# taylorlu/voicepuppet

Measured on AMD Instinct MI355X. Metric: PixReferNet G+D step frames/sec @256x256 bs=32, higher is better.
Workload: dtype bf16; 1 GPU; PixReferNet G+D training step (G + 3xD + VGG16-conv3_3 perceptual + TF-Adam x2), 256x256, ngf=ndf=64, global batch 32 = 32 per GPU; global_batch=32, per_gpu_batch=32, parallelism=dp1

## Files before the change

### include/vp_hip.h

```cpp
#ifndef VP_HIP_H_
#define VP_HIP_H_

#include <stddef.h>
#include <stdint.h>

#ifdef __cplusplus
extern "C" {
#endif

enum vp_status { VP_OK = 0, VP_ERR_ARG = -1, VP_ERR_HIP = -2, VP_ERR_WORKSPACE = -3, VP_ERR_STATE = -4 };
enum vp_dtype { VP_F32 = 0, VP_BF16 = 1 };
enum vp_act { VP_ACT_NONE = 0, VP_ACT_LRELU = 1, VP_ACT_RELU = 2, VP_ACT_TANH = 3, VP_ACT_SIGMOID = 4, VP_ACT_RELU6 = 5, VP_ACT_LEAKY = 6 };

int vp_version(void);
const char* vp_last_error(void);

typedef struct vp_pixrefer_desc {
  int batch;
  int height;
  int ngf, ndf;
  int dtype;
  int training;
  float l1_weight;
  float gan_weight;
// ... 511 lines not shown
typedef struct vp_avimux vp_avimux_t;
size_t vp_avimux_workspace_bytes(const vp_avimux_desc* d);
size_t vp_avimux_out_capacity(const vp_avimux_desc* d);
size_t vp_avimux_table_bytes(const vp_avimux_desc* d, int frames);
int vp_avimux_create(const vp_avimux_desc* d, void* workspace, size_t workspace_bytes, vp_avimux_t** out);
int vp_avimux_segment(vp_avimux_t* h, const unsigned char* data, size_t row_bytes, const int* lengths, const int* frame_slot, int frames,
                      const float* pcm, const int* sample_offset, const int* sample_count, int samples, unsigned char* out, size_t out_capacity,
                      void* stream);
void vp_avimux_destroy(vp_avimux_t* h);

#define VP_TRIPTYCH_MAX_FRAMES 4096
#define VP_TRIPTYCH_MAX_SIZE 1024
typedef struct vp_triptych_desc {
  uint32_t struct_bytes;
  int32_t max_frames;
  int32_t size;
  int32_t face_size;
  int32_t max_side;
} vp_triptych_desc;
size_t vp_triptych_desc_size(void);
typedef struct vp_triptych vp_triptych_t;
size_t vp_triptych_workspace_bytes(const vp_triptych_desc* d);
int vp_triptych_create(const vp_triptych_desc* d, void* workspace, size_t workspace_bytes, void* stream, vp_triptych_t** out);
int vp_triptych_build(vp_triptych_t* h, const unsigned char* frames, const unsigned char* render, const unsigned char* face_mask, const int* geometry,
                      const unsigned char* alpha, int n, unsigned char* triptych, int* status, void* stream);
int vp_triptych_mask(vp_triptych_t* h, const unsigned char* face_mask, const int* geometry, int n, int fill, void* stream);
int vp_triptych_fill_holes(const unsigned char* masks, int n, int height, int width, unsigned char* out, void* stream);
int vp_triptych_blur_taps(int q[21]);
int vp_triptych_tensor(vp_triptych_t* h, const char* name, void** ptr, int64_t shape[4]);
void vp_triptych_destroy(vp_triptych_t* h);

#define VP_KEYMATTE_MAX_FRAMES 4096
#define VP_KEYMATTE_MAX_SIZE 1024
#define VP_KEYMATTE_MAX_RADIUS 16
#define VP_KEYMATTE_MODEL_DOUBLES 19
typedef struct vp_keymatte_desc {
  uint32_t struct_bytes;
  int32_t max_frames;
  int32_t max_height;
  int32_t max_width;
  int32_t max_radius;
} vp_keymatte_desc;
size_t vp_keymatte_desc_size(void);
typedef struct vp_keymatte vp_keymatte_t;
size_t vp_keymatte_workspace_bytes(const vp_keymatte_desc* d);
int vp_keymatte_create(const vp_keymatte_desc* d, void* workspace, size_t workspace_bytes, vp_keymatte_t** out);
void vp_keymatte_destroy(vp_keymatte_t* h);
int vp_keymatte_fit(vp_keymatte_t* h, const unsigned char* frames, size_t row_pitch, size_t frame_stride, int n, int height, int width,
                    int band, int side_rows, double trim, double sigma_min, void* stream);
int vp_keymatte_apply(vp_keymatte_t* h, const unsigned char* frames, size_t row_pitch, size_t frame_stride, int n, int height, int width,
                      double lo, double hi, int radius, double eps, unsigned char* raw, unsigned char* matte, void* stream);
int vp_keymatte_get_model(vp_keymatte_t* h, double* model, void* stream);
int vp_keymatte_set_model(vp_keymatte_t* h, const double* model, void* stream);
int vp_keymatte_tensor(vp_keymatte_t* h, const char* name, void** ptr, int64_t shape[4]);
int vp_keymatte_solve_host(const int64_t moments[21], double sigma_min, double* model);

int vp_key_foreground(vp_keymatte_t* h, const unsigned char* frames, size_t row_pitch, size_t frame_stride, int n, int height, int width,
                      const unsigned char* matte, double despill, unsigned char* out, void* stream);

#define VP_MATTECLEAN_MAX_FRAMES 4096
#define VP_MATTECLEAN_MAX_SIZE 1024
#define VP_MATTECLEAN_MAX_GROW 16
#define VP_MATTECLEAN_MAX_ANCHORS 256
#define VP_MATTECLEAN_REPORT_INTS 8
#define VP_MATTECLEAN_KEEP_ALL 0
#define VP_MATTECLEAN_KEEP_ANCHORED 1
typedef struct vp_matteclean_desc {
  uint32_t struct_bytes;
  int32_t max_frames;
  int32_t max_height;
  int32_t max_width;
} vp_matteclean_desc;
size_t vp_matteclean_desc_size(void);
typedef struct vp_matteclean vp_matteclean_t;
size_t vp_matteclean_workspace_bytes(const vp_matteclean_desc* d);
int vp_matteclean_create(const vp_matteclean_desc* d, void* workspace, size_t workspace_bytes, vp_matteclean_t** out);
void vp_matteclean_destroy(vp_matteclean_t* h);
int vp_matteclean_clean(vp_matteclean_t* h, const unsigned char* matte, int n, int height, int width, int support, int core, int min_area,
                        int max_hole, int grow, int keep, const int* anchors, int k, unsigned char* out, void* stream);
int vp_matteclean_tensor(vp_matteclean_t* h, const char* name, void** ptr, int64_t shape[4]);

unsigned vp_crc32c(const void* data, size_t n, unsigned crc);

#ifdef __cplusplus
}
#endif
#endif
```

### voicepuppet_amd/_lib.py

```python
import ctypes
import os

_HERE = os.path.dirname(os.path.abspath(__file__))
LIB_PATH = os.environ.get("VP_LIB", os.path.join(_HERE, "libvp_hip.so"))

VP_F32, VP_BF16 = 0, 1
ACT_NONE, ACT_LRELU, ACT_RELU, ACT_TANH, ACT_SIGMOID = 0, 1, 2, 3, 4
BN_PATH_PLANNER, BN_PATH_TWO_PASS, BN_PATH_ONE_LAUNCH = 0, 1, 2


class PixReferDesc(ctypes.Structure):
  _fields_ = [("batch", ctypes.c_int), ("height", ctypes.c_int), ("ngf", ctypes.c_int), ("ndf", ctypes.c_int),
              ("dtype", ctypes.c_int), ("training", ctypes.c_int), ("l1_weight", ctypes.c_float),
              ("gan_weight", ctypes.c_float), ("per_sample_bn", ctypes.c_int),
              ("streams", ctypes.c_int), ("d_backward_fork", ctypes.c_int), ("d_beside_vgg", ctypes.c_int)]


class ConvDesc(ctypes.Structure):
  _fields_ = [("kind", ctypes.c_int), ("n", ctypes.c_int), ("h", ctypes.c_int), ("w", ctypes.c_int),
              ("cin", ctypes.c_int), ("cout", ctypes.c_int), ("ksize", ctypes.c_int), ("stride", ctypes.c_int),
              ("pad", ctypes.c_int), ("dtype", ctypes.c_int), ("in_act", ctypes.c_int), ("out_act", ctypes.c_int)]


class LogMelDesc(ctypes.Structure):
# ... 67 lines not shown
  _fields_ = [("struct_bytes", ctypes.c_uint32), ("max_frames", ctypes.c_int32), ("max_height", ctypes.c_int32), ("max_width", ctypes.c_int32)]


FRAME_METRICS_MAX_FRAMES = 4096


class AviMuxDesc(ctypes.Structure):
  _fields_ = [("struct_bytes", ctypes.c_uint32), ("max_frames", ctypes.c_int32), ("row_bytes", ctypes.c_int32), ("slots", ctypes.c_int32),
              ("max_samples", ctypes.c_int32)]


AVIMUX_MAX_FRAMES, AVIMUX_MAX_SLOTS = 4096, 128


class KeyMatteDesc(ctypes.Structure):
  _fields_ = [("struct_bytes", ctypes.c_uint32), ("max_frames", ctypes.c_int32), ("max_height", ctypes.c_int32), ("max_width", ctypes.c_int32),
              ("max_radius", ctypes.c_int32)]


KEYMATTE_MAX_FRAMES, KEYMATTE_MAX_SIZE, KEYMATTE_MAX_RADIUS, KEYMATTE_MODEL_DOUBLES = 4096, 1024, 16, 19


class MatteCleanDesc(ctypes.Structure):
  _fields_ = [("struct_bytes", ctypes.c_uint32), ("max_frames", ctypes.c_int32), ("max_height", ctypes.c_int32), ("max_width", ctypes.c_int32)]


MATTECLEAN_MAX_FRAMES, MATTECLEAN_MAX_SIZE, MATTECLEAN_MAX_GROW, MATTECLEAN_MAX_ANCHORS, MATTECLEAN_REPORT_INTS = 4096, 1024, 16, 256, 8
MATTECLEAN_KEEP_ALL, MATTECLEAN_KEEP_ANCHORED = 0, 1


class TriptychDesc(ctypes.Structure):
  _fields_ = [("struct_bytes", ctypes.c_uint32), ("max_frames", ctypes.c_int32), ("size", ctypes.c_int32), ("face_size", ctypes.c_int32),
              ("max_side", ctypes.c_int32)]


TRIPTYCH_MAX_FRAMES, TRIPTYCH_MAX_SIZE = 4096, 1024


class BfmObserveOpts(ctypes.Structure):
  _fields_ = [("struct_bytes", ctypes.c_uint32), ("visibility", ctypes.c_int32), ("raster_scale", ctypes.c_int32), ("prefilter", ctypes.c_int32),
              ("depth_tol", ctypes.c_float)]


class BfmModel(ctypes.Structure):
  _fields_ = [("nver", ctypes.c_int), ("ntri", ctypes.c_int), ("meanshape", ctypes.c_void_p), ("idBase", ctypes.c_void_p),
              ("exBase", ctypes.c_void_p), ("meantex", ctypes.c_void_p), ("texBase", ctypes.c_void_p), ("tri", ctypes.c_void_p),
              ("point_buf", ctypes.c_void_p), ("center", ctypes.c_double * 3), ("focal", ctypes.c_double),
              ("image_center", ctypes.c_double), ("sh", ctypes.c_double * 5)]


_P = ctypes.c_void_p
_SIGNATURES = {
    "vp_version": (ctypes.c_int, []),
    "vp_last_error": (ctypes.c_char_p, []),
    "vp_pixrefer_param_count": (ctypes.c_size_t, [ctypes.POINTER(PixReferDesc), ctypes.c_int]),
    "vp_pixrefer_param_info": (ctypes.c_int, [ctypes.POINTER(PixReferDesc), ctypes.c_int, ctypes.c_int, ctypes.c_char_p,
                                              ctypes.c_int, ctypes.POINTER(ctypes.c_size_t), ctypes.POINTER(ctypes.c_int),
                                              ctypes.POINTER(ctypes.c_int64)]),
    "vp_pixrefer_workspace_bytes": (ctypes.c_size_t, [ctypes.POINTER(PixReferDesc)]),
    "vp_pixrefer_validate_plan": (ctypes.c_int, [ctypes.POINTER(PixReferDesc)]),
    "vp_pixrefer_create": (ctypes.c_int, [ctypes.POINTER(PixReferDesc), _P, ctypes.c_size_t, _P, _P, _P, _P, _P, _P,
                                          ctypes.POINTER(_P)]),
    "vp_pixrefer_destroy": (None, [_P]),
    "vp_pixrefer_params_changed": (ctypes.c_int, [_P]),
    "vp_pixrefer_optimizer_stepped": (ctypes.c_int, [_P]),
    "vp_pixrefer_forward": (ctypes.c_int, [_P, _P, _P, _P, _P, _P]),
    "vp_pixrefer_forward_fg3": (ctypes.c_int, [_P, _P, _P, _P, _P]),
    "vp_pixrefer_desc_size": (ctypes.c_size_t, []),
    "vp_pixrefer_backward": (ctypes.c_int, [_P, _P]),
    "vp_pixrefer_backward_update": (ctypes.c_int, [_P, _P, _P, _P, _P, ctypes.c_int, ctypes.c_int, ctypes.c_float, ctypes.c_float,
                                                   ctypes.c_float, ctypes.c_float, _P]),
    "vp_pixrefer_backward_d": (ctypes.c_int, [_P, _P]),
    "vp_pixrefer_backward_g": (ctypes.c_int, [_P, _P]),
    "vp_pixrefer_backward_d_fork": (ctypes.c_int, [_P, _P]),
    "vp_pixrefer_backward_d_join": (ctypes.c_int, [_P, _P]),
    "vp_pixrefer_backward_g_stages": (ctypes.c_int, []),
    "vp_pixrefer_backward_g_stage": (ctypes.c_int, [_P, ctypes.c_int, _P]),
    "vp_pixrefer_side_stream": (ctypes.c_void_p, [_P]),
    "vp_pixrefer_use_streams": (ctypes.c_int, [_P, ctypes.c_int]),
    "vp_pixrefer_set_option": (ctypes.c_int, [_P, ctypes.c_char_p, ctypes.c_int]),
    "vp_pixrefer_fetch": (ctypes.c_int, [_P, ctypes.c_int, _P, _P]),
    "vp_pixrefer_counter": (ctypes.c_longlong, [_P, ctypes.c_char_p]),
    "vp_crc32c": (ctypes.c_uint, [_P, ctypes.c_size_t, ctypes.c_uint]),
    "vp_pixrefer_phase_ms": (ctypes.c_int, [_P, ctypes.POINTER(ctypes.c_float), ctypes.c_int]),
    "vp_grad_pack_bf16": (ctypes.c_int, [_P, _P, ctypes.c_size_t, _P]),
    "vp_grad_unpack_bf16": (ctypes.c_int, [_P, _P, ctypes.c_size_t, ctypes.c_float, _P]),
    "vp_pixrefer_update_bucket": (ctypes.c_int, [_P, ctypes.c_int, ctypes.c_int, _P, _P, ctypes.c_int, ctypes.c_float, ctypes.c_float, ctypes.c_float,
                                                 ctypes.c_float, _P]),
    "vp_resize_paste_workspace_bytes": (ctypes.c_size_t, [ctypes.c_int, ctypes.c_int]),
    "vp_resize_paste_u8": (ctypes.c_int, [_P, ctypes.c_int, ctypes.c_int, ctypes.c_int, ctypes.c_int, ctypes.c_int, ctypes.c_int, _P, ctypes.c_int,
                                          ctypes.c_int, ctypes.c_int, ctypes.c_int, _P, _P]),
    "vp_resize_linear_table": (ctypes.c_int, [ctypes.c_int, ctypes.c_int, ctypes.c_int, _P, _P, _P, _P]),
    "vp_mm_workspace_bytes": (ctypes.c_size_t, [ctypes.c_int, ctypes.c_int, ctypes.c_int]),
    "vp_mm_fwd_f32": (ctypes.c_int, [_P, ctypes.c_int, _P, ctypes.c_int, ctypes.c_int, _P, _P, ctypes.c_int, ctypes.c_int, ctypes.c_int, ctypes.c_int, _P, _P]),
    "vp_mm_bwd_data_f32": (ctypes.c_int, [_P, ctypes.c_int, _P, ctypes.c_int, ctypes.c_int, _P, ctypes.c_int, ctypes.c_int, ctypes.c_int, ctypes.c_int,
                                          ctypes.c_int, _P, _P]),
    "vp_mm_bwd_weight_f32": (ctypes.c_int, [_P, ctypes.c_int, _P, ctypes.c_int, _P, ctypes.c_int, ctypes.c_int, ctypes.c_int, ctypes.c_int, _P, _P]),
    "vp_mm_packed_bytes": (ctypes.c_size_t, [ctypes.c_int, ctypes.c_int, ctypes.c_int, ctypes.c_int]),
    "vp_mm_pack_desc_bytes": (ctypes.c_size_t, []),
    "vp_mm_pack_desc": (ctypes.c_int, [ctypes.c_size_t, ctypes.c_int, ctypes.c_int, ctypes.c_int, ctypes.c_int, ctypes.c_int, ctypes.c_int, ctypes.c_size_t, _P]),
    "vp_mm_pack_table": (ctypes.c_int, [_P, ctypes.c_int, _P, _P, _P]),
    "vp_mm_fwd_f32_packed": (ctypes.c_int, [_P, ctypes.c_int, _P, _P, _P, ctypes.c_int, ctypes.c_int, ctypes.c_int, ctypes.c_int, _P, _P]),
    "vp_mm_bwd_data_f32_packed": (ctypes.c_int, [_P, ctypes.c_int, _P, _P, ctypes.c_int, ctypes.c_int, ctypes.c_int, ctypes.c_int, ctypes.c_int, _P, _P]),
    "vp_pixrefer_mark_ms": (ctypes.c_float, [_P, ctypes.c_int, ctypes.c_int]),
    "vp_profile_enable": (ctypes.c_int, [ctypes.c_int]),
    "vp_tune": (ctypes.c_int, [ctypes.c_char_p, ctypes.c_int]),
    "vp_reserve_streams": (ctypes.c_int, []),
    "vp_host_stream": (ctypes.c_void_p, []),
    "vp_pixrefer_pack_frames": (ctypes.c_int, [_P, _P, _P, ctypes.c_int, ctypes.c_int, _P, _P, _P, _P, _P]),
    "vp_profile_collect": (ctypes.c_size_t, [ctypes.c_char_p, ctypes.c_size_t]),
    "vp_pixrefer_tensor": (ctypes.c_int, [_P, ctypes.c_char_p, ctypes.POINTER(_P), ctypes.POINTER(ctypes.c_int64),
                                          ctypes.POINTER(ctypes.c_int)]),
    "vp_adam_tf": (ctypes.c_int, [_P, _P, _P, _P, ctypes.c_size_t, ctypes.c_int, ctypes.c_float, ctypes.c_float,
                                  ctypes.c_float, ctypes.c_float, _P]),
    "vp_conv_workspace_bytes": (ctypes.c_size_t, [ctypes.POINTER(ConvDesc)]),
    "vp_conv_fwd": (ctypes.c_int, [ctypes.POINTER(ConvDesc), _P, _P, _P, _P, _P, _P, _P, _P]),
    "vp_conv_bwd_data": (ctypes.c_int, [ctypes.POINTER(ConvDesc), _P, _P, _P, _P, _P]),
    "vp_conv_bwd_weight": (ctypes.c_int, [ctypes.POINTER(ConvDesc), _P, _P, _P, _P, _P, _P, _P]),
    "vp_conv3x3_c64_bwd_data_pooled_workspace_bytes": (ctypes.c_size_t, [ctypes.POINTER(ConvDesc)]),
    "vp_conv3x3_c64_bwd_data_pooled": (ctypes.c_int, [ctypes.POINTER(ConvDesc), _P, _P, _P, _P, _P, _P, ctypes.c_int, _P]),
    "vp_bn_workspace_bytes": (ctypes.c_size_t, [ctypes.c_int, ctypes.c_int, ctypes.c_int]),
    "vp_bn_stats": (ctypes.c_int, [_P, ctypes.c_int, ctypes.c_int, ctypes.c_int, _P, _P, ctypes.c_float, _P, _P, _P, _P, _P, _P]),
    "vp_logmel_workspace_bytes": (ctypes.c_size_t, [ctypes.POINTER(LogMelDesc)]),
    "vp_logmel_frames": (ctypes.c_int, [ctypes.POINTER(LogMelDesc)]),
    "vp_logmel_create": (ctypes.c_int, [ctypes.POINTER(LogMelDesc), _P, ctypes.c_size_t, _P, ctypes.POINTER(_P)]),
    "vp_logmel_destroy": (None, [_P]),
    "vp_logmel_forward": (ctypes.c_int, [_P, _P, _P, _P]),
    "vp_bfmnet_param_count": (ctypes.c_size_t, []),
    "vp_bfmnet_param_info": (ctypes.c_int, [ctypes.c_int, ctypes.c_char_p, ctypes.c_int, ctypes.POINTER(ctypes.c_size_t),
                                            ctypes.POINTER(ctypes.c_int), ctypes.POINTER(ctypes.c_int64)]),
    "vp_bfmnet_workspace_bytes": (ctypes.c_size_t, [ctypes.POINTER(BfmNetDesc)]),
    "vp_bfmnet_create": (ctypes.c_int, [ctypes.POINTER(BfmNetDesc), _P, ctypes.c_size_t, _P, _P, ctypes.POINTER(_P)]),
    "vp_bfmnet_destroy": (None, [_P]),
    "vp_bfmnet_params_changed": (ctypes.c_int, [_P]),
    "vp_bfmnet_forward": (ctypes.c_int, [_P, _P, _P, _P, _P, _P]),
    "vp_bfmnet_set_decoder_dropout": (ctypes.c_int, [_P, _P, _P]),
    "vp_bfmnet_tensor": (ctypes.c_int, [_P, ctypes.c_char_p, ctypes.POINTER(_P), ctypes.POINTER(ctypes.c_int64)]),
    "vp_bfmstream_desc_size": (ctypes.c_size_t, []),
    "vp_bfmstream_context": (ctypes.c_int, [ctypes.POINTER(BfmStreamDesc)] + [ctypes.POINTER(ctypes.c_int)] * 5),
    "vp_bfmstream_frames_after": (ctypes.c_longlong, [ctypes.POINTER(BfmStreamDesc), ctypes.c_longlong, ctypes.c_int]),
    "vp_bfmstream_workspace_bytes": (ctypes.c_size_t, [ctypes.POINTER(BfmStreamDesc)]),
    "vp_bfmstream_create": (ctypes.c_int, [ctypes.POINTER(BfmStreamDesc), _P, ctypes.c_size_t, _P, _P, ctypes.POINTER(_P)]),
    "vp_bfmstream_destroy": (None, [_P]),
    "vp_bfmstream_params_changed": (ctypes.c_int, [_P]),
    "vp_bfmstream_reset": (ctypes.c_int, [_P, _P]),
    "vp_bfmstream_ready": (ctypes.c_int, [_P, ctypes.c_longlong]),
    "vp_bfmstream_ready_finish": (ctypes.c_int, [_P]),
    "vp_bfmstream_push": (ctypes.c_int, [_P, _P, ctypes.c_longlong, _P, _P, _P]),
    "vp_bfmstream_finish": (ctypes.c_int, [_P, _P, _P, _P]),
    "vp_bfmstream_tensor": (ctypes.c_int, [_P, ctypes.c_char_p, ctypes.POINTER(_P), ctypes.POINTER(ctypes.c_int64)]),
    "vp_bfmstream_group_desc_size": (ctypes.c_size_t, []),
    "vp_puppet_desc_size": (ctypes.c_size_t, []),
    "vp_puppet_workspace_bytes": (ctypes.c_size_t, [ctypes.POINTER(PuppetDesc)]),
    "vp_puppet_create": (ctypes.c_int, [ctypes.POINTER(PuppetDesc), _P, ctypes.c_size_t, _P, ctypes.POINTER(_P)]),
    "vp_puppet_destroy": (None, [_P]),
    "vp_puppet_attach": (ctypes.c_int, [_P, ctypes.c_int, _P, _P, _P, ctypes.c_int, ctypes.c_int, ctypes.c_int, _P]),
    "vp_puppet_set_backgrounds": (ctypes.c_int, [_P, _P, ctypes.c_int]),
    "vp_puppet_splice": (ctypes.c_int, [_P, _P, ctypes.c_int, _P, ctypes.c_int, _P, _P]),
    "vp_puppet_condition": (ctypes.c_int, [_P, _P, ctypes.c_int, _P, ctypes.c_int, _P, _P, _P, _P]),
    "vp_puppet_tensor": (ctypes.c_int, [_P, ctypes.c_char_p, ctypes.POINTER(_P), ctypes.POINTER(ctypes.c_int64)]),
    "vp_puppet_slot_info": (ctypes.c_int, [_P, ctypes.c_int, ctypes.POINTER(ctypes.c_int)]),
    "vp_jpeg_desc_size": (ctypes.c_size_t, []),
    "vp_jpeg_workspace_bytes": (ctypes.c_size_t, [ctypes.POINTER(JpegDesc)]),
    "vp_jpeg_frame_capacity": (ctypes.c_size_t, [ctypes.POINTER(JpegDesc)]),
    "vp_jpeg_create": (ctypes.c_int, [ctypes.POINTER(JpegDesc), _P, ctypes.c_size_t, _P, ctypes.POINTER(_P)]),
    "vp_jpeg_encode": (ctypes.c_int, [_P, _P, ctypes.c_int, _P, ctypes.c_size_t, _P, _P]),
# ... 236 lines not shown
```

### voicepuppet_amd/csrc/wgrad_tr.hip

```cpp
#include <stdlib.h>

#include "conv_ops.h"
#include "igemm_device.h"
#include "launch.h"

namespace vp {

__device__ __forceinline__ int tr_swz(int p) { return ((p & 3) | (((p >> 3) & 1) << 2)) << 1; }

typedef short v4s16 __attribute__((ext_vector_type(4)));

template <int ROWB>
__device__ __forceinline__ uint4 tr_frag8(const char* __restrict__ stage, int off) {
  typedef __attribute__((address_space(3))) v4s16 lds_v4;
  const v4s16 lo = __builtin_amdgcn_ds_read_tr16_b64_v4i16((lds_v4*)(stage + off));
  const v4s16 hi = __builtin_amdgcn_ds_read_tr16_b64_v4i16((lds_v4*)(stage + off + 4 * ROWB));
  union { v4s16 v[2]; uint4 u; } f;
  f.v[0] = lo; f.v[1] = hi;
  return f.u;
}

struct TrTask {
  const bf16* base;
  int C;
  int s, dh, dw;
  int Hs, Ws;
  int p;
  bool ok;
};

__device__ __forceinline__ TrTask tr_task(const PixSrc& src, int ch, bool ok, int s, int dh, int dw, int Hs, int Ws, int p, const void* zeros) {
  TrTask t;
  const bool second = ch >= src.C[0];
  t.C = second ? src.C[1] : src.C[0];
  t.base = reinterpret_cast<const bf16*>(second ? src.ptr[1] : src.ptr[0]) + (second ? ch - src.C[0] : ch);
  t.s = s; t.dh = dh; t.dw = dw; t.Hs = Hs; t.Ws = Ws; t.p = p; t.ok = ok;
  if (!ok) { t.base = reinterpret_cast<const bf16*>(zeros); t.C = 0; }
  return t;
}

__device__ __forceinline__ const void* tr_src(const WgradArgs& a, const TrTask& t, int it) {
  const int slot = it * 32 + t.p;
  const int r = slot & ((1 << a.lw) - 1), q = (slot >> a.lw) & ((1 << a.lh) - 1), n = slot >> (a.lw + a.lh);
  const int ih = q * t.s + t.dh, iw = r * t.s + t.dw;
  const bool ok = t.ok && n < a.N && q < a.Hb && r < a.Wb && (unsigned)ih < (unsigned)t.Hs && (unsigned)iw < (unsigned)t.Ws;
  return ok ? (const void*)(t.base + ((size_t)(n * t.Hs + ih) * t.Ws + iw) * t.C) : a.zeros;
}

template <int WM, int WN, int TC, int TP, int NST, bool FAST, bool EXACT = false>
__global__ __launch_bounds__(WM * WN * 64, (TC * TP > 16 ? 2 : 4)) void wgrad_tr_kernel(const WgradArgs a) {
  constexpr int NW = WM * WN;
  static_assert(NW == 8, "eight waves");
  constexpr int BM = WM * TC * 16, BN = WN * TP * 16;
  constexpr int PA = BM / 8, PB = BN / 8;
  constexpr int ASTG = 32 * PA, BSTG = 32 * PB, STG = ASTG + BSTG;
  constexpr int JA = ASTG / 64 / NW, JB = BSTG / 64 / NW;
  static_assert(JA * NW * 64 == ASTG && JB * NW * 64 == BSTG, "whole DMA instructions per wave");
  constexpr int J = JA + JB;
  extern __shared__ __attribute__((aligned(16))) char smem[];
  uint4* lds = reinterpret_cast<uint4*>(smem);

  const int tid = threadIdx.x, lane = tid & 63;
  const int wave = __builtin_amdgcn_readfirstlane(tid >> 6);
  int bx = blockIdx.x, by = blockIdx.y, bz = blockIdx.z;
  if (a.xcd_remap && (gridDim.z & 7) == 0) {
    const int ntile = gridDim.x * gridDim.y;
    const int L = bx + by * gridDim.x + bz * ntile;
    const int xcd = L & 7, j = L >> 3;
    bz = xcd + 8 * (j / ntile);
    const int t = j % ntile;
    bx = t % gridDim.x; by = t / gridDim.x;
  }
  const int m_base = bx * BM, d_base = by * BN, split = bz;
  const int niter = (a.N << (a.lw + a.lh)) / 32;
  const int per = (niter + a.splitk - 1) / a.splitk;
  const int it0 = split * per, it1 = min(niter, it0 + per);

  TrTask ta[JA], tb[JB];
#pragma unroll
  for (int j = 0; j < JA; ++j) {
    const int idx = (wave + NW * j) * 64 + lane;
    const int p = idx / PA, c = (idx % PA) ^ tr_swz(p);
    const int m = m_base + c * 8;
    const int tap = m >> a.log2Gc, ch = m & a.gc_mask;
    int tdh = 0, tdw = 0;
#pragma unroll
    for (int t = 0; t < 16; ++t) if (t == tap) { tdh = a.taps.dh[t]; tdw = a.taps.dw[t]; }
    ta[j] = tr_task(a.g, ch, tap < a.ntaps && ch < a.g.C[0] + a.g.C[1], a.s, tdh, tdw, a.Hgin, a.Wgin, p, a.zeros);
  }
#pragma unroll
  for (int j = 0; j < JB; ++j) {
    const int idx = (wave + NW * j) * 64 + lane;
    const int p = idx / PB, c = (idx % PB) ^ tr_swz(p);
    const int ch = d_base + c * 8;
    tb[j] = tr_task(a.d, ch, ch < a.Dc, 1, 0, 0, a.Hb, a.Wb, p, a.zeros);
  }
  const int W2 = 1 << a.lw;
  const bool gsecond = a.g.C[1] > 0 && (m_base & (a.Gc - 1)) >= a.g.C[0];
  const bool dsecond = a.d.C[1] > 0 && d_base >= a.d.C[0];
  const int gC = gsecond ? a.g.C[1] : a.g.C[0], dC = dsecond ? a.d.C[1] : a.d.C[0];
  constexpr bool fast = FAST;
  const unsigned gguard = (unsigned)((2 * a.Wgin + 2) * gC * 2);
  __amdgpu_buffer_rsrc_t rsG = make_rsrc((const char*)(gsecond ? a.g.ptr[1] : a.g.ptr[0]) - gguard,
                                         (unsigned)((size_t)a.N * a.Hgin * a.Wgin * gC * 2) + gguard);
  __amdgpu_buffer_rsrc_t rsD = make_rsrc(dsecond ? a.d.ptr[1] : a.d.ptr[0], (unsigned)((size_t)a.N * a.Hb * a.Wb * dC * 2));
  int fq[JA], fB[JA], fr[JA], fD[JA];
  unsigned fvo[JA];
  bool fok[JA];
  int bq[JB], br[JB];
  unsigned bvo[JB];
  bool bok[JB];
#pragma unroll
  for (int j = 0; j < JA; ++j) {
    const TrTask& t = ta[j];
    const int pq = W2 <= 32 ? t.p >> a.lw : 0, pr = W2 <= 32 ? t.p & (W2 - 1) : t.p;
    fq[j] = pq; fB[j] = pq * t.s + t.dh; fr[j] = pr; fD[j] = pr * t.s + t.dw;
    const int chl = (int)(t.base - reinterpret_cast<const bf16*>(gsecond ? a.g.ptr[1] : a.g.ptr[0]));
    fvo[j] = gguard + (unsigned)(((fB[j] * a.Wgin + fD[j]) * gC + chl) * 2);
    fok[j] = t.ok;
    if (EXACT && !t.ok) fvo[j] = DMA_OOB;
  }
#pragma unroll
  for (int j = 0; j < JB; ++j) {
    const TrTask& t = tb[j];
    bq[j] = W2 <= 32 ? t.p >> a.lw : 0; br[j] = W2 <= 32 ? t.p & (W2 - 1) : t.p;
    const int chl = (int)(t.base - reinterpret_cast<const bf16*>(dsecond ? a.d.ptr[1] : a.d.ptr[0]));
    bvo[j] = (unsigned)(((bq[j] * a.Wb + br[j]) * dC + chl) * 2);
    bok[j] = t.ok;
    if (EXACT && !t.ok) bvo[j] = DMA_OOB;
  }
  auto issue_fast = [&](int it, int stage) {
    uint4* la = lds + stage * STG;
    uint4* lb = la + ASTG;
    const int u = it * 32;
    const int ru = u & (W2 - 1), qu = (u >> a.lw) & ((1 << a.lh) - 1), nu = u >> (a.lw + a.lh);
    const bool nok = nu < a.N;
    const unsigned gso = (unsigned)((((nu * a.Hgin + qu * a.s) * a.Wgin + ru * a.s) * gC) * 2);
    const unsigned dso = (unsigned)((((nu * a.Hb + qu) * a.Wb + ru) * dC) * 2);
    const int qs = qu * a.s, rs = ru * a.s;
    if constexpr (EXACT) {
#pragma unroll
      for (int j = 0; j < JA; ++j) {
        const bool ok = (unsigned)(qs + fB[j]) < (unsigned)a.Hgin && (unsigned)(rs + fD[j]) < (unsigned)a.Wgin;
        dma16_buf(rsG, ok ? fvo[j] : DMA_OOB, gso, la + (wave + NW * j) * 64);
      }
#pragma unroll
      for (int j = 0; j < JB; ++j) dma16_buf(rsD, bvo[j], dso, lb + (wave + NW * j) * 64);
    } else {
#pragma unroll
      for (int j = 0; j < JA; ++j) {
        const bool ok = fok[j] && nok && qu + fq[j] < a.Hb && ru + fr[j] < a.Wb &&
                        (unsigned)(qs + fB[j]) < (unsigned)a.Hgin && (unsigned)(rs + fD[j]) < (unsigned)a.Wgin;
        dma16_buf(rsG, ok ? fvo[j] : DMA_OOB, gso, la + (wave + NW * j) * 64);
      }
#pragma unroll
      for (int j = 0; j < JB; ++j) {
        const bool ok = bok[j] && nok && qu + bq[j] < a.Hb && ru + br[j] < a.Wb;
        dma16_buf(rsD, ok ? bvo[j] : DMA_OOB, dso, lb + (wave + NW * j) * 64);
      }
    }
  };
  auto issue = [&](int it, int stage) {
    if constexpr (fast) { issue_fast(it, stage); return; }
    uint4* la = lds + stage * STG;
    uint4* lb = la + ASTG;
#pragma unroll
    for (int j = 0; j < JA; ++j) dma16(tr_src(a, ta[j], it), la + (wave + NW * j) * 64);
#pragma unroll
    for (int j = 0; j < JB; ++j) dma16(tr_src(a, tb[j], it), lb + (wave + NW * j) * 64);
  };

  const int wm = wave / WN, wn = wave - wm * WN;
  const int g = lane >> 4, t16 = lane & 15;
  const int fp = 8 * g + (t16 >> 2), q2 = t16 & 3, fsw = tr_swz(fp);
  int offA[TC], offB[TP];
#pragma unroll
  for (int tc = 0; tc < TC; ++tc) offA[tc] = fp * (BM * 2) + (((2 * (wm * TC + tc) + (q2 >> 1)) ^ fsw) << 4) + (q2 & 1) * 8;
#pragma unroll
  for (int tp = 0; tp < TP; ++tp) offB[tp] = ASTG * 16 + fp * (BN * 2) + (((2 * (wn * TP + tp) + (q2 >> 1)) ^ fsw) << 4) + (q2 & 1) * 8;

  f32x4 acc[TC][TP];
#pragma unroll
  for (int i = 0; i < TC; ++i)
#pragma unroll
    for (int j = 0; j < TP; ++j) acc[i][j] = (f32x4){0.f, 0.f, 0.f, 0.f};

  if (it0 < it1) {
#pragma unroll
    for (int dd = 0; dd < NST - 1; ++dd) if (it0 + dd < it1) issue(it0 + dd, dd);
    int st = 0;
    for (int it = it0; it < it1; ++it) {
      if (it + NST - 2 < it1) asm volatile("s_waitcnt vmcnt(%0)" ::"n"((NST - 2) * J) : "memory");
      else asm volatile("s_waitcnt vmcnt(0)" ::: "memory");
      __builtin_amdgcn_s_barrier();
      asm volatile("" ::: "memory");
      const int stn = st == 0 ? NST - 1 : st - 1;
      if (it + NST - 1 < it1) issue(it + NST - 1, stn);
      const char* stage = smem + (size_t)st * STG * 16;
      uint4 fa[TC], fb[TP];
#pragma unroll
      for (int tp = 0; tp < TP; ++tp) fb[tp] = tr_frag8<BN * 2>(stage, offB[tp]);
#pragma unroll
      for (int tc = 0; tc < TC; ++tc) fa[tc] = tr_frag8<BM * 2>(stage, offA[tc]);
#pragma unroll
      for (int tc = 0; tc < TC; ++tc)
#pragma unroll
        for (int tp = 0; tp < TP; ++tp) acc[tc][tp] = mma16<bf16>(fa[tc], fb[tp], acc[tc][tp]);
      st = st == NST - 1 ? 0 : st + 1;
    }
  }

  if (a.splitk == 1) {
#pragma unroll
    for (int tc = 0; tc < TC; ++tc)
#pragma unroll
      for (int tp = 0; tp < TP; ++tp) {
        const int m0 = m_base + (wm * TC + tc) * 16 + 4 * (lane >> 4);
        const int d = d_base + (wn * TP + tp) * 16 + (lane & 15);
        if (d >= a.Dreal) continue;
#pragma unroll
        for (int e = 0; e < 4; ++e) {
          const int m = m0 + e, tap = m >> a.log2Gc, gc = m & a.gc_mask;
          if (tap < a.ntaps && gc < a.Greal) {
            float* o = a.dW + ((size_t)tap * a.Greal + gc) * a.Dreal + d;
            *o = acc[tc][tp][e] + (a.accumulate ? *o : 0.f);
          }
        }
      }
    return;
  }
#pragma unroll
  for (int tc = 0; tc < TC; ++tc)
#pragma unroll
    for (int tp = 0; tp < TP; ++tp) {
      const int m0 = m_base + (wm * TC + tc) * 16 + 4 * (lane >> 4);
      const int d = d_base + (wn * TP + tp) * 16 + (lane & 15);
      float* pp = a.partial + ((size_t)split * a.Mpad + m0) * a.Dpad + d;
#pragma unroll
      for (int e = 0; e < 4; ++e) pp[(size_t)e * a.Dpad] = acc[tc][tp][e];
    }
}

template <int WM, int WN, int TC, int TP>
static hipError_t launch_wgrad_tr_t(const WgradArgs& a, hipStream_t st, const char** variant) {
  constexpr int NST = 3;
  constexpr int BM = WM * TC * 16, BN = WN * TP * 16;
  const size_t smem = (size_t)NST * 32 * (BM / 8 + BN / 8) * 16;
  dim3 grid(a.Mpad / BM, a.Dpad / BN, a.splitk);
  WgradArgs b = a;
  const size_t gbytes = (size_t)a.N * a.Hgin * a.Wgin * (a.g.C[0] > a.g.C[1] ? a.g.C[0] : a.g.C[1]) * 2;
  const size_t dbytes = (size_t)a.N * a.Hb * a.Wb * (a.d.C[0] > a.d.C[1] ? a.d.C[0] : a.d.C[1]) * 2;
  bool fast = gbytes < 0x60000000ull && dbytes < 0x60000000ull && a.lw + a.lh >= 5;
  if (a.g.C[1] > 0) fast = fast && a.Gc >= BM && a.g.C[0] % BM == 0;
  if (a.d.C[1] > 0) fast = fast && a.d.C[0] % BN == 0;
  b.fast_tr = fast ? 1 : 0;
  b.xcd_remap = 1;
  const bool exact = fast && a.Hb == (1 << a.lh) && a.Wb == (1 << a.lw);
  if (variant) *variant = exact ? "tr_exact" : fast ? "tr_fast" : "tr";
  auto kern = exact ? wgrad_tr_kernel<WM, WN, TC, TP, NST, true, true> : fast ? wgrad_tr_kernel<WM, WN, TC, TP, NST, true> : wgrad_tr_kernel<WM, WN, TC, TP, NST, false>;
  (void)hipFuncSetAttribute((const void*)kern, hipFuncAttributeMaxDynamicSharedMemorySize, (int)smem);
  hipLaunchKernelGGL(kern, grid, dim3(512), smem, st, b);
  return hipGetLastError();
}

hipError_t launch_wgrad_tr(const WgradArgs& a, hipStream_t st, const char** variant, int* tile_cols) {
  if (tile_cols) *tile_cols = 128;
  if (wgrad_big_knob() && a.Mpad % 256 == 0 && a.Dpad % 256 == 0 && (long long)(a.Mpad / 256) * (a.Dpad / 256) * a.splitk >= 256 &&
      (a.d.C[1] == 0 || a.d.C[0] % 256 == 0) && a.lw + a.lh >= 5) {
    if (tile_cols) *tile_cols = 256;
    return launch_wgrad_tr_t<4, 2, 4, 8>(a, st, variant);
  }
  if (a.Mpad % 256 == 0) return launch_wgrad_tr_t<4, 2, 4, 4>(a, st, variant);
  return launch_wgrad_tr_t<4, 2, 2, 4>(a, st, variant);
}

}
```

Baseline: 4533 frames/s.

## Restructure wgrad_tr main loop into unrolled ring schedule skipping invalid chunks

Replaces the weight-gradient transpose kernel's runtime-indexed pipeline loop with a compile-time-unrolled ring of stages. LDS fragment reads use immediate offsets and finely staged lgkmcnt waits so MFMAs can start before all fragments arrive. The fast path walks only valid spatial chunks with incremental address steps, skipping chunks that fall entirely in padding. The old loop is kept for the 16-tile non-fast config. The change adds code size and register pressure, plus a host-side schedule export for testing.

```diff
diff --git a/include/vp_hip.h b/include/vp_hip.h
--- a/include/vp_hip.h
+++ b/include/vp_hip.h
@@ -617,6 +617,8 @@
 
 unsigned vp_crc32c(const void* data, size_t n, unsigned crc);
 
+int vp_wgrad_tr_schedule(int niter, int splitk, int split, int lw, int lh, int hb, int* events, int cap);
+
 #ifdef __cplusplus
 }
 #endif
diff --git a/voicepuppet_amd/_lib.py b/voicepuppet_amd/_lib.py
--- a/voicepuppet_amd/_lib.py
+++ b/voicepuppet_amd/_lib.py
@@ -173,6 +173,7 @@
     "vp_pixrefer_fetch": (ctypes.c_int, [_P, ctypes.c_int, _P, _P]),
     "vp_pixrefer_counter": (ctypes.c_longlong, [_P, ctypes.c_char_p]),
     "vp_crc32c": (ctypes.c_uint, [_P, ctypes.c_size_t, ctypes.c_uint]),
+    "vp_wgrad_tr_schedule": (ctypes.c_int, [ctypes.c_int] * 6 + [ctypes.POINTER(ctypes.c_int), ctypes.c_int]),
     "vp_pixrefer_phase_ms": (ctypes.c_int, [_P, ctypes.POINTER(ctypes.c_float), ctypes.c_int]),
     "vp_grad_pack_bf16": (ctypes.c_int, [_P, _P, ctypes.c_size_t, _P]),
     "vp_grad_unpack_bf16": (ctypes.c_int, [_P, _P, ctypes.c_size_t, ctypes.c_float, _P]),
diff --git a/voicepuppet_amd/csrc/wgrad_tr.hip b/voicepuppet_amd/csrc/wgrad_tr.hip
--- a/voicepuppet_amd/csrc/wgrad_tr.hip
+++ b/voicepuppet_amd/csrc/wgrad_tr.hip
@@ -1,10 +1,19 @@
 #include <stdlib.h>
+
+#include <type_traits>
 
 #include "conv_ops.h"
 #include "igemm_device.h"
 #include "launch.h"
+#include "wgrad_tr_sched.h"
 
 namespace vp {
+
+#ifdef VP_WGTR_PARENT_LOOP
+#define VP_WGTR_PARENT_LOOP_ALL true
+#else
+#define VP_WGTR_PARENT_LOOP_ALL false
+#endif
 
 __device__ __forceinline__ int tr_swz(int p) { return ((p & 3) | (((p >> 3) & 1) << 2)) << 1; }
 
@@ -18,6 +27,21 @@
   union { v4s16 v[2]; uint4 u; } f;
   f.v[0] = lo; f.v[1] = hi;
   return f.u;
+}
+
+typedef unsigned u32x2 __attribute__((ext_vector_type(2)));
+struct TrFrag { u32x2 lo, hi; };
+template <int ROWB, int IMM>
+__device__ __forceinline__ TrFrag tr_frag8a(unsigned addr) {
+  TrFrag f;
+  asm volatile("ds_read_b64_tr_b16 %0, %1 offset:%2" : "=v"(f.lo) : "v"(addr), "n"(IMM));
+  asm volatile("ds_read_b64_tr_b16 %0, %1 offset:%2" : "=v"(f.hi) : "v"(addr), "n"(IMM + 4 * ROWB));
+  return f;
+}
+template <int PENDING> __device__ __forceinline__ void tr_frag_wait() { asm volatile("s_waitcnt lgkmcnt(%0)" ::"n"(PENDING > 15 ? 15 : PENDING) : "memory"); }
+__device__ __forceinline__ uint4 tr_frag_get(TrFrag& f) {
+  asm volatile("" : "+v"(f.lo)); asm volatile("" : "+v"(f.hi));
+  return make_uint4(f.lo.x, f.lo.y, f.hi.x, f.hi.y);
 }
 
 struct TrTask {
@@ -57,6 +81,7 @@
   constexpr int JA = ASTG / 64 / NW, JB = BSTG / 64 / NW;
   static_assert(JA * NW * 64 == ASTG && JB * NW * 64 == BSTG, "whole DMA instructions per wave");
   constexpr int J = JA + JB;
+  constexpr bool PARENT = VP_WGTR_PARENT_LOOP_ALL || (!FAST && TC * TP == 16);
   extern __shared__ __attribute__((aligned(16))) char smem[];
   uint4* lds = reinterpret_cast<uint4*>(smem);
 
@@ -73,8 +98,8 @@
   }
   const int m_base = bx * BM, d_base = by * BN, split = bz;
   const int niter = (a.N << (a.lw + a.lh)) / 32;
-  const int per = (niter + a.splitk - 1) / a.splitk;
-  const int it0 = split * per, it1 = min(niter, it0 + per);
+  int it0, it1;
+  tr_split_range(niter, a.splitk, split, it0, it1);
 
   TrTask ta[JA], tb[JB];
 #pragma unroll
@@ -129,47 +154,6 @@
     bok[j] = t.ok;
     if (EXACT && !t.ok) bvo[j] = DMA_OOB;
   }
-  auto issue_fast = [&](int it, int stage) {
-    uint4* la = lds + stage * STG;
-    uint4* lb = la + ASTG;
-    const int u = it * 32;
-    const int ru = u & (W2 - 1), qu = (u >> a.lw) & ((1 << a.lh) - 1), nu = u >> (a.lw + a.lh);
-    const bool nok = nu < a.N;
-    const unsigned gso = (unsigned)((((nu * a.Hgin + qu * a.s) * a.Wgin + ru * a.s) * gC) * 2);
-    const unsigned dso = (unsigned)((((nu * a.Hb + qu) * a.Wb + ru) * dC) * 2);
-    const int qs = qu * a.s, rs = ru * a.s;
-    if constexpr (EXACT) {
-#pragma unroll
-      for (int j = 0; j < JA; ++j) {
-        const bool ok = (unsigned)(qs + fB[j]) < (unsigned)a.Hgin && (unsigned)(rs + fD[j]) < (unsigned)a.Wgin;
-        dma16_buf(rsG, ok ? fvo[j] : DMA_OOB, gso, la + (wave + NW * j) * 64);
-      }
-#pragma unroll
-      for (int j = 0; j < JB; ++j) dma16_buf(rsD, bvo[j], dso, lb + (wave + NW * j) * 64);
-    } else {
-#pragma unroll
-      for (int j = 0; j < JA; ++j) {
-        const bool ok = fok[j] && nok && qu + fq[j] < a.Hb && ru + fr[j] < a.Wb &&
-                        (unsigned)(qs + fB[j]) < (unsigned)a.Hgin && (unsigned)(rs + fD[j]) < (unsigned)a.Wgin;
-        dma16_buf(rsG, ok ? fvo[j] : DMA_OOB, gso, la + (wave + NW * j) * 64);
-      }
-#pragma unroll
-      for (int j = 0; j < JB; ++j) {
-        const bool ok = bok[j] && nok && qu + bq[j] < a.Hb && ru + br[j] < a.Wb;
-        dma16_buf(rsD, ok ? bvo[j] : DMA_OOB, dso, lb + (wave + NW * j) * 64);
-      }
-    }
-  };
-  auto issue = [&](int it, int stage) {
-    if constexpr (fast) { issue_fast(it, stage); return; }
-    uint4* la = lds + stage * STG;
-    uint4* lb = la + ASTG;
-#pragma unroll
-    for (int j = 0; j < JA; ++j) dma16(tr_src(a, ta[j], it), la + (wave + NW * j) * 64);
-#pragma unroll
-    for (int j = 0; j < JB; ++j) dma16(tr_src(a, tb[j], it), lb + (wave + NW * j) * 64);
-  };
-
   const int wm = wave / WN, wn = wave - wm * WN;
   const int g = lane >> 4, t16 = lane & 15;
   const int fp = 8 * g + (t16 >> 2), q2 = t16 & 3, fsw = tr_swz(fp);
@@ -185,29 +169,198 @@
 #pragma unroll
     for (int j = 0; j < TP; ++j) acc[i][j] = (f32x4){0.f, 0.f, 0.f, 0.f};
 
-  if (it0 < it1) {
-#pragma unroll
-    for (int dd = 0; dd < NST - 1; ++dd) if (it0 + dd < it1) issue(it0 + dd, dd);
-    int st = 0;
-    for (int it = it0; it < it1; ++it) {
-      if (it + NST - 2 < it1) asm volatile("s_waitcnt vmcnt(%0)" ::"n"((NST - 2) * J) : "memory");
-      else asm volatile("s_waitcnt vmcnt(0)" ::: "memory");
+  if constexpr (PARENT) {
+    auto issue_fast = [&](int it, int stage) {
+      uint4* la = lds + stage * STG;
+      uint4* lb = la + ASTG;
+      const int u = it * 32;
+      const int ru = u & (W2 - 1), qu = (u >> a.lw) & ((1 << a.lh) - 1), nu = u >> (a.lw + a.lh);
+      const bool nok = nu < a.N;
+      const unsigned gso = (unsigned)((((nu * a.Hgin + qu * a.s) * a.Wgin + ru * a.s) * gC) * 2);
+      const unsigned dso = (unsigned)((((nu * a.Hb + qu) * a.Wb + ru) * dC) * 2);
+      const int qs = qu * a.s, rs = ru * a.s;
+      if constexpr (EXACT) {
+#pragma unroll
+        for (int j = 0; j < JA; ++j) {
+          const bool ok = (unsigned)(qs + fB[j]) < (unsigned)a.Hgin && (unsigned)(rs + fD[j]) < (unsigned)a.Wgin;
+          dma16_buf(rsG, ok ? fvo[j] : DMA_OOB, gso, la + (wave + NW * j) * 64);
+        }
+#pragma unroll
+        for (int j = 0; j < JB; ++j) dma16_buf(rsD, bvo[j], dso, lb + (wave + NW * j) * 64);
+      } else {
+#pragma unroll
+        for (int j = 0; j < JA; ++j) {
+          const bool ok = fok[j] && nok && qu + fq[j] < a.Hb && ru + fr[j] < a.Wb &&
+                          (unsigned)(qs + fB[j]) < (unsigned)a.Hgin && (unsigned)(rs + fD[j]) < (unsigned)a.Wgin;
+          dma16_buf(rsG, ok ? fvo[j] : DMA_OOB, gso, la + (wave + NW * j) * 64);
+        }
+#pragma unroll
+        for (int j = 0; j < JB; ++j) {
+          const bool ok = bok[j] && nok && qu + bq[j] < a.Hb && ru + br[j] < a.Wb;
+          dma16_buf(rsD, ok ? bvo[j] : DMA_OOB, dso, lb + (wave + NW * j) * 64);
+        }
+      }
+    };
+    auto issue = [&](int it, int stage) {
+      if constexpr (fast) { issue_fast(it, stage); return; }
+      uint4* la = lds + stage * STG;
+      uint4* lb = la + ASTG;
+#pragma unroll
+      for (int j = 0; j < JA; ++j) dma16(tr_src(a, ta[j], it), la + (wave + NW * j) * 64);
+#pragma unroll
+      for (int j = 0; j < JB; ++j) dma16(tr_src(a, tb[j], it), lb + (wave + NW * j) * 64);
+    };
+    if (it0 < it1) {
+#pragma unroll
+      for (int dd = 0; dd < NST - 1; ++dd) if (it0 + dd < it1) issue(it0 + dd, dd);
+      int st = 0;
+      for (int it = it0; it < it1; ++it) {
+        if (it + NST - 2 < it1) asm volatile("s_waitcnt vmcnt(%0)" ::"n"((NST - 2) * J) : "memory");
+        else asm volatile("s_waitcnt vmcnt(0)" ::: "memory");
+        __builtin_amdgcn_s_barrier();
+        asm volatile("" ::: "memory");
+        const int stn = st == 0 ? NST - 1 : st - 1;
+        if (it + NST - 1 < it1) issue(it + NST - 1, stn);
+        const char* stage = smem + (size_t)st * STG * 16;
+        uint4 fa[TC], fb[TP];
+#pragma unroll
+        for (int tp = 0; tp < TP; ++tp) fb[tp] = tr_frag8<BN * 2>(stage, offB[tp]);
+#pragma unroll
+        for (int tc = 0; tc < TC; ++tc) fa[tc] = tr_frag8<BM * 2>(stage, offA[tc]);
+#pragma unroll
+        for (int tc = 0; tc < TC; ++tc)
+#pragma unroll
+          for (int tp = 0; tp < TP; ++tp) acc[tc][tp] = mma16<bf16>(fa[tc], fb[tp], acc[tc][tp]);
+        st = st == NST - 1 ? 0 : st + 1;
+      }
+    }
+  } else {
+    int n_chunks = it0 < it1 ? it1 - it0 : 0;
+    int itn = it0;
+    TrOrigin o = {0, 0, 0};
+    int dq = 1, Hv = 0;
+    unsigned gso = 0, dso = 0, gstep = 0, grow = 0, gimg = 0, dstep = 0, drow = 0, dimg = 0;
+    if constexpr (fast) {
+      const int lcpi = a.lw + a.lh - 5;
+      const bool wide = W2 >= 32;
+      int vpi;
+      tr_walk(a.lw, a.lh, EXACT ? 1 << a.lh : a.Hb, dq, vpi, Hv);
+      if (it0 < it1) n_chunks = tr_valid_before(it1, lcpi, vpi) - tr_valid_before(it0, lcpi, vpi);
+      o.set(tr_first_valid(it0, lcpi, vpi), a.lw, a.lh);
+      const int ru = o.ru, qu = o.qu, nu = o.nu;
+      gso = (unsigned)((((nu * a.Hgin + qu * a.s) * a.Wgin + ru * a.s) * gC) * 2);
+      dso = (unsigned)((((nu * a.Hb + qu) * a.Wb + ru) * dC) * 2);
+      gstep = (unsigned)((wide ? 32 * a.s : dq * a.s * a.Wgin) * gC * 2);
+      grow = wide ? (unsigned)((a.s * a.Wgin - W2 * a.s) * gC * 2) : 0u;
+      gimg = (unsigned)((a.Hgin - Hv * a.s) * a.Wgin * gC * 2);
+      dstep = (unsigned)((wide ? 32 : dq * a.Wb) * dC * 2);
+      drow = wide ? (unsigned)((a.Wb - W2) * dC * 2) : 0u;
+      dimg = (unsigned)((a.Hb - Hv) * a.Wb * dC * 2);
+    }
+    auto issue = [&](auto stage_c) {
+      constexpr int stage = decltype(stage_c)::value;
+      uint4* la = lds + stage * STG;
+      uint4* lb = la + ASTG;
+      if constexpr (!fast) {
+#pragma unroll
+        for (int j = 0; j < JA; ++j) dma16(tr_src(a, ta[j], itn), la + (wave + NW * j) * 64);
+#pragma unroll
+        for (int j = 0; j < JB; ++j) dma16(tr_src(a, tb[j], itn), lb + (wave + NW * j) * 64);
+        ++itn;
+      } else {
+        const int ru = o.ru, qu = o.qu, nu = o.nu;
+        const int qs = qu * a.s, rs = ru * a.s;
+        if constexpr (EXACT) {
+#pragma unroll
+          for (int j = 0; j < JA; ++j) {
+            const bool ok = (unsigned)(qs + fB[j]) < (unsigned)a.Hgin && (unsigned)(rs + fD[j]) < (unsigned)a.Wgin;
+            dma16_buf(rsG, ok ? fvo[j] : DMA_OOB, gso, la + (wave + NW * j) * 64);
+          }
+#pragma unroll
+          for (int j = 0; j < JB; ++j) dma16_buf(rsD, bvo[j], dso, lb + (wave + NW * j) * 64);
+        } else {
+          const bool nok = nu < a.N;
+#pragma unroll
+          for (int j = 0; j < JA; ++j) {
+            const bool ok = fok[j] && nok && qu + fq[j] < a.Hb && ru + fr[j] < a.Wb &&
+                            (unsigned)(qs + fB[j]) < (unsigned)a.Hgin && (unsigned)(rs + fD[j]) < (unsigned)a.Wgin;
+            dma16_buf(rsG, ok ? fvo[j] : DMA_OOB, gso, la + (wave + NW * j) * 64);
+          }
+#pragma unroll
+          for (int j = 0; j < JB; ++j) {
+            const bool ok = bok[j] && nok && qu + bq[j] < a.Hb && ru + br[j] < a.Wb;
+            dma16_buf(rsD, ok ? bvo[j] : DMA_OOB, dso, lb + (wave + NW * j) * 64);
+          }
+        }
+        bool wr, wq;
+        o.advance(W2, dq, Hv, wr, wq);
+        gso += gstep + (wr ? grow : 0u) + (wq ? gimg : 0u);
+        dso += dstep + (wr ? drow : 0u) + (wq ? dimg : 0u);
+      }
+    };
+    constexpr int STGB = STG * 16;
+    constexpr int IMM_MAX = 0xFFFF - 4 * (BM > BN ? BM : BN) * 2;
+    static_assert((NST - 2) * STGB <= IMM_MAX, "all stages but the last within the DS offset field");
+    constexpr bool LAST_REG = (NST - 1) * STGB > IMM_MAX;
+    const unsigned lds0 = (unsigned)(size_t)(__attribute__((address_space(3))) char*)smem;
+    unsigned adA[TC], adB[TP], adAl[LAST_REG ? TC : 1], adBl[LAST_REG ? TP : 1];
+#pragma unroll
+    for (int tc = 0; tc < TC; ++tc) {
+      adA[tc] = lds0 + offA[tc]; asm volatile("" : "+v"(adA[tc]));
+      if constexpr (LAST_REG) { adAl[tc] = adA[tc] + (NST - 1) * STGB; asm volatile("" : "+v"(adAl[tc])); }
+    }
+#pragma unroll
+    for (int tp = 0; tp < TP; ++tp) {
+      adB[tp] = lds0 + offB[tp]; asm volatile("" : "+v"(adB[tp]));
+      if constexpr (LAST_REG) { adBl[tp] = adB[tp] + (NST - 1) * STGB; asm volatile("" : "+v"(adBl[tp])); }
+    }
+
+    tr_static_steps([&](auto dd) { if (decltype(dd)::value < n_chunks) issue(dd); }, std::make_integer_sequence<int, NST - 1>{});
+    tr_ring_schedule<NST>(n_chunks, [&](auto stage_c, auto ahead_c, auto issue_c) {
+      asm volatile("s_waitcnt vmcnt(%0)" ::"n"(decltype(ahead_c)::value * J) : "memory");
       __builtin_amdgcn_s_barrier();
       asm volatile("" ::: "memory");
-      const int stn = st == 0 ? NST - 1 : st - 1;
-      if (it + NST - 1 < it1) issue(it + NST - 1, stn);
-      const char* stage = smem + (size_t)st * STG * 16;
-      uint4 fa[TC], fb[TP];
-#pragma unroll
-      for (int tp = 0; tp < TP; ++tp) fb[tp] = tr_frag8<BN * 2>(stage, offB[tp]);
-#pragma unroll
-      for (int tc = 0; tc < TC; ++tc) fa[tc] = tr_frag8<BM * 2>(stage, offA[tc]);
-#pragma unroll
-      for (int tc = 0; tc < TC; ++tc)
-#pragma unroll
-        for (int tp = 0; tp < TP; ++tp) acc[tc][tp] = mma16<bf16>(fa[tc], fb[tp], acc[tc][tp]);
-      st = st == NST - 1 ? 0 : st + 1;
-    }
+      TrFrag ra[TC], rb[TP];
+      auto rdA = [&](auto tci) {
+        constexpr int tc = decltype(tci)::value;
+        if constexpr (std::is_same_v<decltype(stage_c), int>) ra[tc] = tr_frag8a<BM * 2, 0>(adA[tc] + (unsigned)stage_c * STGB);
+        else if constexpr (LAST_REG && decltype(stage_c)::value == NST - 1) ra[tc] = tr_frag8a<BM * 2, 0>(adAl[tc]);
+        else ra[tc] = tr_frag8a<BM * 2, decltype(stage_c)::value * STGB>(adA[tc]);
+      };
+      auto rdB = [&](auto tpi) {
+        constexpr int tp = decltype(tpi)::value;
+        if constexpr (std::is_same_v<decltype(stage_c), int>) rb[tp] = tr_frag8a<BN * 2, 0>(adB[tp] + (unsigned)stage_c * STGB);
+        else if constexpr (LAST_REG && decltype(stage_c)::value == NST - 1) rb[tp] = tr_frag8a<BN * 2, 0>(adBl[tp]);
+        else rb[tp] = tr_frag8a<BN * 2, decltype(stage_c)::value * STGB>(adB[tp]);
+      };
+      if constexpr (!std::is_same_v<decltype(stage_c), int>) {
+        if constexpr (decltype(issue_c)::value) issue(std::integral_constant<int, (decltype(stage_c)::value + NST - 1) % NST>{});
+      } else {
+        static_assert(!decltype(issue_c)::value, "the tail issues nothing");
+      }
+      if constexpr (!fast) __builtin_amdgcn_sched_barrier(0);
+      rdA(std::integral_constant<int, 0>{});
+      tr_static_steps(rdB, std::make_integer_sequence<int, TP>{});
+      tr_static_steps([&](auto tci) { if constexpr (decltype(tci)::value > 0) rdA(tci); }, std::make_integer_sequence<int, TC>{});
+      uint4 fb[TP];
+      tr_static_steps([&](auto tci) {
+        constexpr int tc = decltype(tci)::value;
+        if constexpr (tc > 0) tr_frag_wait<2 * (TC - 1 - tc)>();
+        const uint4 fa = tc > 0 ? tr_frag_get(ra[tc]) : make_uint4(0, 0, 0, 0);
+        tr_static_steps([&](auto tpi) {
+          constexpr int tp = decltype(tpi)::value;
+          if constexpr (tc == 0) {
+            tr_frag_wait<2 * (TC - 1) + 2 * (TP - 1 - tp)>();
+            fb[tp] = tr_frag_get(rb[tp]);
+            acc[0][tp] = mma16<bf16>(tr_frag_get(ra[0]), fb[tp], acc[0][tp]);
+            __builtin_amdgcn_sched_barrier(0);
+          } else {
+            acc[tc][tp] = mma16<bf16>(fa, fb[tp], acc[tc][tp]);
+          }
+        }, std::make_integer_sequence<int, TP>{});
+        __builtin_amdgcn_sched_barrier(0);
+      }, std::make_integer_sequence<int, TC>{});
+    });
   }
 
   if (a.splitk == 1) {
@@ -275,3 +428,33 @@
 }
 
 }
+
+extern "C" int vp_wgrad_tr_schedule(int niter, int splitk, int split, int lw, int lh, int hb, int* events, int cap) {
+  using namespace vp;
+  constexpr int NST = 3;
+  int count = 0;
+  auto emit = [&](int op, int x, int y, int z) {
+    if (count < cap) { events[4 * count] = op; events[4 * count + 1] = x; events[4 * count + 2] = y; events[4 * count + 3] = z; }
+    ++count;
+  };
+  int it0, it1, dq, vpi, Hv;
+  tr_split_range(niter, splitk, split, it0, it1);
+  const int lcpi = lw + lh - 5;
+  tr_walk(lw, lh, hb, dq, vpi, Hv);
+  const int n_chunks = it0 < it1 ? tr_valid_before(it1, lcpi, vpi) - tr_valid_before(it0, lcpi, vpi) : 0;
+  TrOrigin o;
+  o.set(tr_first_valid(it0, lcpi, vpi), lw, lh);
+  auto issue = [&](int stage) {
+    emit(0, ((o.nu << lh) + o.qu) * (1 << lw) / 32 + o.ru / 32, stage, o.nu << 20 | o.qu << 10 | o.ru);
+    bool wr, wq;
+    o.advance(1 << lw, dq, Hv, wr, wq);
+  };
+  tr_static_steps([&](auto dd) { if (decltype(dd)::value < n_chunks) issue(dd); }, std::make_integer_sequence<int, NST - 1>{});
+  tr_ring_schedule<NST>(n_chunks, [&](auto stage_c, auto ahead_c, auto issue_c) {
+    const int stage = stage_c;
+    emit(1, decltype(ahead_c)::value, 0, 0);
+    if (decltype(issue_c)::value) issue((stage + NST - 1) % NST);
+    emit(2, stage, 0, 0);
+  });
+  return count;
+}
diff --git a/voicepuppet_amd/csrc/wgrad_tr_sched.h b/voicepuppet_amd/csrc/wgrad_tr_sched.h
--- /dev/null
+++ b/voicepuppet_amd/csrc/wgrad_tr_sched.h
@@ -0,0 +1,72 @@
+#pragma once
+#include <utility>
+
+#if defined(__HIPCC__) || defined(__CUDACC__)
+#define VP_SCHED_HD __host__ __device__ __forceinline__
+#else
+#define VP_SCHED_HD inline
+#endif
+
+namespace vp {
+
+template <typename F, int... Is> VP_SCHED_HD void tr_static_steps(F&& f, std::integer_sequence<int, Is...>) {
+  (f(std::integral_constant<int, Is>{}), ...);
+}
+
+VP_SCHED_HD void tr_split_range(int niter, int splitk, int split, int& it0, int& it1) {
+  const int per = (niter + splitk - 1) / splitk;
+  it0 = split * per;
+  it1 = niter < it0 + per ? niter : it0 + per;
+}
+
+VP_SCHED_HD int tr_valid_before(int x, int lcpi, int vpi) {
+  const int in = x & ((1 << lcpi) - 1);
+  return (x >> lcpi) * vpi + (in < vpi ? in : vpi);
+}
+VP_SCHED_HD int tr_first_valid(int x, int lcpi, int vpi) { return (x & ((1 << lcpi) - 1)) < vpi ? x : ((x >> lcpi) + 1) << lcpi; }
+
+struct TrOrigin {
+  int ru, qu, nu;
+  VP_SCHED_HD void set(int chunk, int lw, int lh) {
+    const int u = chunk * 32;
+    ru = u & ((1 << lw) - 1); qu = (u >> lw) & ((1 << lh) - 1); nu = u >> (lw + lh);
+  }
+  VP_SCHED_HD void advance(int W2, int dq, int Hv, bool& wr, bool& wq) {
+    ru += 32;
+    wr = ru >= W2;
+    ru = wr ? 0 : ru; qu += wr ? dq : 0;
+    wq = qu >= Hv;
+    qu = wq ? 0 : qu; nu += wq ? 1 : 0;
+  }
+};
+VP_SCHED_HD void tr_walk(int lw, int lh, int Hb, int& dq, int& vpi, int& Hv) {
+  const bool wide = lw >= 5;
+  dq = wide ? 1 : 32 >> lw;
+  const int cpi = 1 << (lw + lh - 5);
+  const int v = wide ? Hb << (lw - 5) : (Hb + dq - 1) >> (5 - lw);
+  vpi = v < cpi ? v : cpi;
+  Hv = wide ? vpi >> (lw - 5) : vpi * dq;
+}
+
+template <int NST> VP_SCHED_HD constexpr int tr_ring_prologue(int n) { return n < NST - 1 ? n : NST - 1; }
+
+template <int NST, typename F> VP_SCHED_HD void tr_ring_schedule(int n, F&& step) {
+  static_assert(NST >= 2, "a ring of at least two stages");
+  const int tail = tr_ring_prologue<NST>(n);
+  const int trips = (n - tail) / NST, rest = (n - tail) - trips * NST;
+  for (int t = 0; t < trips; ++t)
+    tr_static_steps([&](auto s) { step(s, std::integral_constant<int, NST - 2>{}, std::true_type{}); }, std::make_integer_sequence<int, NST>{});
+  tr_static_steps([&](auto s) {
+    if (decltype(s)::value < rest) step(s, std::integral_constant<int, NST - 2>{}, std::true_type{});
+  }, std::make_integer_sequence<int, NST - 1>{});
+  int stage = rest;
+  tr_static_steps([&](auto i) {
+    constexpr int AHEAD = NST - 2 - decltype(i)::value;
+    if (tail > AHEAD) {
+      step(stage, std::integral_constant<int, AHEAD>{}, std::false_type{});
+      stage = stage == NST - 1 ? 0 : stage + 1;
+    }
+  }, std::make_integer_sequence<int, NST - 1>{});
+}
+
+}
```

Measured after the change: 4540 frames/s, median of 4. No clear change (+0.2%).
